# zhoupengwei/tloam

Hardware: AMD Instinct MI355X
Metric: gauss_newton_iters_per_sec (higher is better)
Workload: dtype f64

## Files before the change

tloam_amd/csrc/tl_gn.hip:

```cpp
#include <stdlib.h>
#include <string.h>

#include <hip/hip_ext.h>

#include "tl_common.hpp"
#include "tl_finish.hpp"

namespace tl {

struct Acc {
  double v[27];
  double pm;
  int pe;
};

__host__ __device__ constexpr int ut(int i, int j) { return i * 6 - (i * (i - 1)) / 2 + (j - i); }

__device__ __forceinline__ double fast_rcp(double x) {
  double r = __builtin_amdgcn_rcp(x);
  return __builtin_fma(r, __builtin_fma(-x, r, 1.0), r);
}
__device__ __forceinline__ double fast_rsqrt(double x) {
  double y = __builtin_amdgcn_rsq(x);
  const double h = 0.5 * x * y;
// ... 688 lines not shown
__device__ __forceinline__ void load_state_words(const GnState* st, GnState* sm) {
  constexpr int kWords = (int)(sizeof(GnState) / 8);
  static_assert(kWords <= 256, "one word per thread");
  if (threadIdx.x < kWords)
    reinterpret_cast<unsigned long long*>(sm)[threadIdx.x] = reinterpret_cast<const unsigned long long*>(st)[threadIdx.x];
}
__device__ __forceinline__ void stop_comm_error(GnState* st) {
  if (threadIdx.x == 0) { st->done = 1; st->comm_error = 1; }
}
__device__ __forceinline__ bool mbox_receive(const MboxView& mb, unsigned long long id, double* out , int count, int lane) {
  const bool ok = mbox_gather(mb, id, out, count, lane);
  if (lane == 0) {
    mb.ctr[0] = id;
    if (!ok) mb.ctr[1] = 1ull;
  }
  return ok;
}
__global__ __launch_bounds__(64) void k_gn_step(GnState* st, const double* __restrict__ in48, unsigned long long* iter_span) {
  __shared__ double tot[kReduceBuf];
  __shared__ double scr[32];
  __shared__ GnState s_in;
  if (threadIdx.x < kReduceBuf) tot[threadIdx.x] = in48[threadIdx.x];
  load_state_lds(st, &s_in, threadIdx.x);
  __syncthreads();
  if (s_in.done) return;
  const bool first = s_in.phase == PH_ITER0;
  gn_consume(st, tot, threadIdx.x, &s_in, scr);
  if (threadIdx.x == 0) iter_span_note(iter_span, first);
}
void launch_gn_step(GnState* st, const double* in48, hipStream_t s, unsigned long long* iter_span) {
  hipLaunchKernelGGL(k_gn_step, dim3(1), dim3(64), 0, s, st, in48, iter_span);
}
__global__ __launch_bounds__(64) void k_gn_step_mbox(GnState* st, MboxView mb, unsigned long long* iter_span) {
  __shared__ double tot[kMboxSlot];
  __shared__ double scr[32];
  __shared__ GnState s_in;
  load_state_lds(st, &s_in, threadIdx.x);
  __syncthreads();
  if (s_in.done) return;
  const bool ok = mbox_receive(mb, mbox_next_id(mb), tot, kReduceBuf, threadIdx.x);
  __syncthreads();
  if (!ok) {
    stop_comm_error(st);
    return;
  }
  const bool first = s_in.phase == PH_ITER0;
  gn_consume(st, tot, threadIdx.x, &s_in, scr);
  if (threadIdx.x == 0) iter_span_note(iter_span, first);
}
void launch_gn_step_mbox(GnState* st, const MboxView& mb, hipStream_t s, unsigned long long* iter_span) {
  hipLaunchKernelGGL(k_gn_step_mbox, dim3(1), dim3(64), 0, s, st, mb, iter_span);
}
__global__ __launch_bounds__(64) void k_mbox_gather_only(double* out48, MboxView mb) {
  __shared__ double tot[kMboxSlot];
  mbox_receive(mb, mbox_next_id(mb), tot, kReduceBuf, threadIdx.x);
  if (threadIdx.x < kReduceBuf) out48[threadIdx.x] = tot[threadIdx.x];
}
void launch_mbox_gather_only(double* out48, const MboxView& mb, hipStream_t s) {
  hipLaunchKernelGGL(k_mbox_gather_only, dim3(1), dim3(64), 0, s, out48, mb);
}
__global__ __launch_bounds__(64) void k_mbox_allreduce(double* buf, int count, MboxView mb) {
  __shared__ double vals[kMboxSlot];
  const int t = threadIdx.x;
  if (t < count) vals[t] = buf[t];
  __syncthreads();
  const unsigned long long id = mbox_next_id(mb);
  mbox_post(mb, id, vals, count, t);
  mbox_receive(mb, id, vals, count, t);
  __syncthreads();
  if (t < count) buf[t] = vals[t];
}
void launch_mbox_allreduce(double* buf, int count, const MboxView& mb, hipStream_t s) {
  hipLaunchKernelGGL(k_mbox_allreduce, dim3(1), dim3(64), 0, s, buf, count, mb);
}

__global__ __launch_bounds__(kRedThreads) void k_reduce_and_step(const double* __restrict__ partials, int rows,
                                                                 GnState* __restrict__ st, unsigned long long* iter_span) {
  __shared__ double lds[8 * 33];
  __shared__ double tot[kReduceBuf];
  __shared__ GnState s_in;
#ifdef TLOAM_STEP_PROFILE
  if (threadIdx.x == 0) st->dbg[0] = (double)__builtin_readcyclecounter();
#endif
  load_state_words(st, &s_in);
#ifdef TLOAM_STEP_PROFILE
  asm volatile("s_waitcnt vmcnt(0)" ::: "memory");
  if (threadIdx.x == 0) st->dbg[7] = (double)__builtin_readcyclecounter();
#endif
  fold_rows<false, 4>(partials, rows, lds, tot);
#ifdef TLOAM_STEP_PROFILE
  if (threadIdx.x == 0) st->dbg[8] = (double)__builtin_readcyclecounter();
#endif
  if (s_in.done) return;
  const bool first = s_in.phase == PH_ITER0;
  if (threadIdx.x < 64) gn_consume(st, tot, threadIdx.x, &s_in, lds );
  if (threadIdx.x == 0) iter_span_note(iter_span, first);
#ifdef TLOAM_STEP_PROFILE
  if (threadIdx.x == 0) st->dbg[6] = (double)__builtin_readcyclecounter();
#endif
}
struct K3Step {
  int* ticket;
  unsigned long long* span;
  unsigned long long* iter_span;
  MboxView mb;
};
template <bool SINGLE, int W = 4>
__global__ __launch_bounds__(64 * W, 2) void k3_sweep_step(const double* __restrict__ seg0, int stride0, int cap0, int unused,
                                                        GnState* __restrict__ st, const int* __restrict__ seg_n,
                                                        double* __restrict__ partials, CorrView cv, K3Step fs) {
  __shared__ double red[W][32];
  __shared__ double s_grp[8 * 33];
  __shared__ double tot[kMboxSlot];
  __shared__ GnState s_in;
  SweepStamps ts;
  sweep_body<SINGLE, W, false>(seg0, stride0, cap0, (unused & 2) != 0 , false, st, seg_n, cv, red,
                               ts, [&] {
    if (fs.span && blockIdx.x == 0 && threadIdx.x == 0)
      __hip_atomic_store(fs.span, (unsigned long long)wall_clock64(), __ATOMIC_RELAXED, __HIP_MEMORY_SCOPE_AGENT);
    load_state_words(st, &s_in);
  }, [&] {
    if (!k3_take_ticket<W>(partials, red, fs.ticket)) return;
    if (fs.span && threadIdx.x == 0) {
      const unsigned long long t1 = wall_clock64();
      const unsigned long long t0 = __hip_atomic_load(fs.span, __ATOMIC_RELAXED, __HIP_MEMORY_SCOPE_AGENT);
      fs.span[1] += t1 - t0;
      fs.span[2] += 1ull;
    }
    fold_rows<true>(partials, (int)gridDim.x, s_grp, tot);
    if (threadIdx.x == 0) __hip_atomic_store(fs.ticket, 0, __ATOMIC_RELAXED, __HIP_MEMORY_SCOPE_AGENT);
    if (threadIdx.x >= 64) return;
    if (fs.mb.nranks > 0) {
      const unsigned long long id = mbox_next_id(fs.mb);
      mbox_post(fs.mb, id, tot, kReduceBuf, (int)threadIdx.x);
      const bool ok = mbox_receive(fs.mb, id, tot, kReduceBuf, (int)threadIdx.x);
      asm volatile("s_waitcnt lgkmcnt(0)" ::: "memory");
      if (!ok) {
        stop_comm_error(st);
        return;
      }
    }
    const bool first = s_in.phase == PH_ITER0;
    gn_consume(st, tot, (int)threadIdx.x, &s_in, s_grp );
    if (threadIdx.x == 0) iter_span_note(fs.iter_span, first);
  });
}
void launch_k3_step(const CorrView& cv, GnState* st, double* partials, int grid, bool single, bool wide, int* ticket, unsigned long long* span,
                    const MboxView* mb_or_null, hipStream_t s, hipEvent_t ev_start, hipEvent_t ev_stop, unsigned long long* iter_span) {
  auto kern = single ? k3_sweep_step<true> : wide ? k3_sweep_step<false, 8> : k3_sweep_step<false>;
  K3Step fs;
  memset(&fs, 0, sizeof(fs));
  fs.ticket = ticket;
  fs.span = span;
  fs.iter_span = iter_span;
  if (mb_or_null) fs.mb = *mb_or_null;
  launch_sweep(kern, grid, wide ? 512 : 256, s, ev_start, ev_stop, cv, 0, st, partials, cv, fs);
}

__global__ __launch_bounds__(256, 1) void k_sweep_step_small(const double* __restrict__ seg0, int stride0, int cap0, int tagged,
                                                             GnState* __restrict__ st, const int* __restrict__ seg_n,
                                                             double* __restrict__ partials, int* __restrict__ ticket,
                                                             CorrView cv, unsigned long long* iter_span) {
  __shared__ double red[4][32];
  __shared__ double s_grp[8 * 33];
  __shared__ double s_rows[kTaggedRows * 28];
  __shared__ double tot[kReduceBuf];
  __shared__ GnState s_in;
  const int lane = threadIdx.x & 63, wave = __builtin_amdgcn_readfirstlane(threadIdx.x >> 6);
  const int gw = blockIdx.x * 4 + wave;
#ifdef TLOAM_STEP_PROFILE
  const unsigned long long c_entry = __builtin_readcyclecounter();
#endif
  ChunkData pre;
  const SingleWork wk = single_work_of(cv, cap0, gw, lane);
  const bool w2 = (tagged & 2) != 0;
  tagged &= 1;
  single_fetch(cv, seg0, stride0, wk, pre, w2);
  {
    constexpr int kWords = (int)(sizeof(GnState) / 8);
    static_assert(kWords <= 256, "one word per thread");
    if (threadIdx.x < kWords)
      reinterpret_cast<unsigned long long*>(&s_in)[threadIdx.x] = reinterpret_cast<const unsigned long long*>(st)[threadIdx.x];
  }
  unsigned long long* const epoch = reinterpret_cast<unsigned long long*>(ticket + 2);
  const unsigned long long epoch0 = *epoch;
  if (st->done) return;
  const Rt T = st->Rt_eval;
#ifdef TLOAM_STEP_PROFILE
  asm volatile("s_waitcnt lgkmcnt(0)" ::: "memory");
  const unsigned long long c_pose = __builtin_readcyclecounter();
#endif
  Acc a;
  sweep_single(cv, seg_n, T, wk, pre, a);
#ifdef TLOAM_STEP_PROFILE
  const unsigned long long c_eval = __builtin_readcyclecounter();
#endif
  const double wtot = wave_reduce_acc(a, lane);
  if ((lane & 1) == 0) red[wave][lane >> 1] = wtot;
  __syncthreads();
#ifdef TLOAM_STEP_PROFILE
  const unsigned long long c_sweep = __builtin_readcyclecounter();
#endif
  if (tagged) {
    k3_post_row_tagged(partials, red, epoch0 + 1ull);
    if (blockIdx.x != 0 || threadIdx.x >= 64) return;
#ifdef TLOAM_STEP_PROFILE
    if (threadIdx.x == 0) {
      st->dbg[7] = (double)c_sweep; st->dbg[0] = (double)__builtin_readcyclecounter();
      st->dbg[8] = (double)c_entry; st->dbg[9] = (double)c_pose; st->dbg[10] = (double)c_eval;
    }
#endif
    const bool ok = poll_fold_tagged(partials, (int)gridDim.x, epoch0 + 1ull, s_rows, tot, (int)threadIdx.x);
    if (threadIdx.x == 0) *epoch = epoch0 + 1ull;
    if (!ok) {
      if (threadIdx.x == 0) { st->done = 1; st->comm_error = 1; }
      return;
    }
  } else {
    if (!k3_take_ticket(partials, red, ticket)) return;
#ifdef TLOAM_STEP_PROFILE
    if (threadIdx.x == 0) { st->dbg[7] = (double)c_sweep; st->dbg[0] = (double)__builtin_readcyclecounter(); }
#endif
    fold_rows<true>(partials, (int)gridDim.x, s_grp, tot);
    if (threadIdx.x == 0) __hip_atomic_store(ticket, 0, __ATOMIC_RELAXED, __HIP_MEMORY_SCOPE_AGENT);
  }
  const bool first = s_in.phase == PH_ITER0;
  if (threadIdx.x < 64) gn_consume(st, tot, threadIdx.x, &s_in, s_grp );
  if (threadIdx.x == 0) iter_span_note(iter_span, first);
#ifdef TLOAM_STEP_PROFILE
  if (threadIdx.x == 0) st->dbg[6] = (double)__builtin_readcyclecounter();
#endif
}
void launch_sweep_step_small(const CorrView& cv, GnState* st, double* partials, int* ticket, int grid, hipStream_t s,
                             unsigned long long* iter_span) {
  launch_sweep(k_sweep_step_small, grid, 256, s, nullptr, nullptr, cv, grid <= kTaggedRows ? 1 : 0 , st, partials, ticket, cv,
               iter_span);
}
#include "tl_prep.hpp"

__device__ __forceinline__ bool weight_out_of_range(const WeightParams& wp, int kind, double c) {
  if (!wp.active[kind]) return false;
  if (c == 0) return false;
  if (c >= wp.th1 || c <= wp.th2) return false;
  if (c < wp.th1 * (1.0 - 1e-9) && c > wp.th2 * (1.0 + 1e-9)) return false;
  const double w = sqrt(wp.noise_bound_sq * wp.mu * (wp.mu + 1) / c) - wp.mu;
  return !(w >= 0.0 && w <= 1.0);
}
constexpr int kExtRowBase = 512;
__device__ __forceinline__ void post_ext_segment(double* __restrict__ partials, int gw, double cs, double bad, int kind, unsigned long long tag,
                                                 int lane, int base_word = kExtRowBase) {
  if (lane >= 8) return;
  unsigned long long wd = 0ull;
  const double cs0 = rdlane(cs, 0), bad0 = rdlane(bad, 0);
  if (lane == 0) wd = (unsigned long long)__double_as_longlong(cs0);
  else if (lane == 1) wd = (unsigned long long)__double_as_longlong(bad0);
  else if (lane == 2) wd = (unsigned long long)(long long)kind;
  const unsigned long long x = xor8(lane < 7 ? seg_word(wd, lane) : 0ull);
  if (lane == 7) wd = check_mix(tag) ^ x;
  __hip_atomic_store(reinterpret_cast<unsigned long long*>(partials) + base_word + (size_t)gw * 8 + lane, wd, __ATOMIC_RELAXED,
                     __HIP_MEMORY_SCOPE_AGENT);
}
__device__ __forceinline__ bool poll_fold_ext(const double* __restrict__ partials, int nwaves, unsigned long long tag, double* s_ext ,
                                              double* fin , int lane, int base_word = kExtRowBase) {
  const bool have = lane >= 1 && lane < nwaves;
  const unsigned long long mtag = check_mix(tag);
  const unsigned long long* p = reinterpret_cast<const unsigned long long*>(partials) + base_word + (size_t)(have ? lane : 1) * 8;
  unsigned long long w[8];
  const unsigned long long t0 = wall_clock64();
  bool ok_all;
  for (unsigned spins = 1;; ++spins) {
#pragma unroll
    for (int i = 0; i < 8; ++i) w[i] = __hip_atomic_load(p + i, __ATOMIC_RELAXED, __HIP_MEMORY_SCOPE_AGENT);
    unsigned long long x = w[7];
#pragma unroll
    for (int i = 0; i < 7; ++i) x ^= seg_word(w[i], i);
    ok_all = __all((!have || x == mtag) ? 1 : 0) != 0;
    if (ok_all) break;
    if ((spins & 63u) == 0 && wall_clock64() - t0 > 100000000ull) break;
    __builtin_amdgcn_s_sleep(1);
  }
  const double cs = have ? __longlong_as_double((long long)w[0]) : 0.0;
  const double bad = have ? __longlong_as_double((long long)w[1]) : 0.0;
  const int kind = have ? (int)(long long)w[2] : -1;
  double t[5];
#pragma unroll
  for (int k = 0; k < 4; ++k) t[k] = kind == k ? cs : 0.0;
  t[4] = bad;
#pragma unroll
  for (int off = 32; off > 0; off >>= 1)
#pragma unroll
    for (int k = 0; k < 5; ++k) t[k] += __shfl_down(t[k], off, 64);
  if (lane == 0) {
#pragma unroll
    for (int k = 0; k < 5; ++k) fin[k] = t[k];
  }
  asm volatile("s_waitcnt lgkmcnt(0)" ::: "memory");
  (void)s_ext;
  return ok_all;
}

__device__ __forceinline__ int finish_by_consumer(GnState* st, GnState* sm , const SolveFinish& F, int oi,
                                                  const double* fin, const int nseg[kKinds], double* sh , int lane,
                                                  bool lead = true) {
  constexpr int kWords = (int)(offsetof(GnState, dbg) / 8);
  const OuterCtl ctl{F.cost_threshold, 1, oi == F.n_iter - 1 ? 1 : 0};
  int next = 4;
  if (!sm->done) {
    if (lane == 0) {
      sm->incomplete = OS_INCOMPLETE;
      sm->stop = 2;
      sm->run_build = sm->run_refresh = 0;
    }
  } else {
    if (lane < 16) {
      double v = 0.0;
      if (lane < 4) v = fin[lane];
      else if (lane < 8) v = (double)(lane == 4 ? nseg[0] : (lane == 5 ? nseg[1] : (lane == 6 ? nseg[2] : nseg[3])));
      else if (lane == 8) v = fin[4];
      sh[lane] = v;
      if (lead) F.sums16[lane] = v;
    }
    asm volatile("s_waitcnt lgkmcnt(0)" ::: "memory");
    publish_and_rearm(sh, sm, lane, ctl);
    asm volatile("s_waitcnt lgkmcnt(0)" ::: "memory");
    next = (sm->stop == 0 && sm->run_build == 0 && sm->run_refresh != 0 && oi + 1 < F.n_iter) ? 3 : 4;
  }
  asm volatile("s_waitcnt lgkmcnt(0)" ::: "memory");
  if (!lead) return next;
  for (int w = lane; w < kWords; w += 64) reinterpret_cast<unsigned long long*>(st)[w] = reinterpret_cast<const unsigned long long*>(sm)[w];
  mirror_wave(sm, F.hm[oi], lane, (sm->stop == 0 && next == 4) ? (int)(sm->incomplete | OS_NEEDS_HOST) : -1);
  if (sm->stop != 0)
    for (int j = oi + 1; j < F.n_iter; ++j) mirror_wave(sm, F.hm[j], lane, (int)OS_SKIPPED);
  return next;
}

constexpr int kAllRowsParity = kTaggedRows * kAccStride;
constexpr int kAllExtBase = 2 * kAllRowsParity;
constexpr int kAllExtParity = 64 * 8;
__device__ __forceinline__ bool next_is_failure(const double* s_msg) {
  asm volatile("s_waitcnt lgkmcnt(0)" ::: "memory");
  return (int)s_msg[12] == 5;
}
__global__ __launch_bounds__(256, 1) void k_solve_all(const double* __restrict__ seg0, int stride0, int cap0, int max_sweeps,
                                                      GnState* __restrict__ st, const int* __restrict__ seg_n,
                                                      double* __restrict__ partials, int* __restrict__ ticket, CorrView cv, SolvePrep prep,
                                                      int* __restrict__ seg_n_out, SolveFinish F) {
  __shared__ double red[4][32];
  __shared__ double s_scr[32];
  __shared__ double s_rows[kTaggedRows * 28];
  __shared__ double s_ext[64 * 3];
  __shared__ double s_fin[8];
  __shared__ double s_sh[16];
  __shared__ double tot[kReduceBuf];
  __shared__ double s_msg[16];
  __shared__ GnState s_in;
  const int lane = threadIdx.x & 63, wave = __builtin_amdgcn_readfirstlane(threadIdx.x >> 6);
  const int gw = blockIdx.x * 4 + wave;
  const bool stepper = wave == 0;
  const bool lead = blockIdx.x == 0;
  const bool self_prep = prep.sv.flagb != nullptr;
  const unsigned long long sabotage = ((max_sweeps >> 16) & 1) ? (1ull << 40) : 0ull;
  max_sweeps &= 0xffff;
  unsigned long long* const epoch = reinterpret_cast<unsigned long long*>(ticket + 2);
#ifdef TLOAM_STEP_PROFILE
  unsigned long long* const prof = reinterpret_cast<unsigned long long*>(partials) + 2048;
  const bool prof_c = lead && stepper && lane == 0;
  const bool prof_p = (int)blockIdx.x == (int)gridDim.x / 2 && wave == 1 && lane == 0;
#define TL_PROF(cond, slot) if (cond) prof[(slot)] = wall_clock64();
#else
#define TL_PROF(cond, slot)
#endif
  ChunkData pre;
  const SingleWork wk = single_work_of(cv, cap0, gw, lane);
  single_fetch(cv, seg0, stride0, wk, pre);
  FlagBytes fbytes;
  if (self_prep && wk.kind >= 0) load_flag_bytes(prep.sv.flagb, wk.kind, lane, fbytes);
  if (stepper) {
    constexpr int kWords = (int)(sizeof(GnState) / 8);
    for (int w = lane; w < kWords; w += 64)
      reinterpret_cast<unsigned long long*>(&s_in)[w] = reinterpret_cast<const unsigned long long*>(st)[w];
  }
  const unsigned long long tag0 = (*epoch + 1ull) << 8;
  int oi = F.first_iter;
  if (F.enabled && (st->stop != 0 || st->next_outer != oi)) return;
  const bool build = self_prep && (!prep.run_build || *prep.run_build != 0);
  const bool refresh = self_prep && !build && prep.run_refresh && *prep.run_refresh != 0;
  const bool done_at_entry = st->done != 0;
  Rt T = st->Rt_eval;
  int n_mine = 0;
  int slot[2] = {0, 0};
  int nseg[kKinds] = {0, 0, 0, 0};
  if (lead && stepper) {
    if (build) {
      FlagBytes fb[kKinds];
#pragma unroll
      for (int k = 0; k < kKinds; ++k) load_flag_bytes(prep.sv.flagb, k, lane, fb[k]);
#pragma unroll
      for (int k = 0; k < kKinds; ++k) nseg[k] = kind_set_of(prep, cv, k, lane, fb[k]).total;
      if (lane < kKinds) seg_n_out[lane] = lane == 0 ? nseg[0] : (lane == 1 ? nseg[1] : (lane == 2 ? nseg[2] : nseg[3]));
    } else {
#pragma unroll
      for (int k = 0; k < kKinds; ++k) nseg[k] = seg_n[k];
    }
  }
  if (wk.kind >= 0) {
    if (build) {
      n_mine = self_compact(prep, cv, wk, lane, fbytes, pre, slot);
    } else {
      n_mine = seg_n[wk.kind];
      if (self_prep) {
        slots_of_chunk(prep, cv, wk, n_mine, slot);
        if (refresh) self_refresh(prep, cv, wk, n_mine, slot, pre);
      }
    }
  }
  if (stepper) {
    asm volatile("s_waitcnt vmcnt(0) lgkmcnt(0)" ::: "memory");
    if (build && lane < 6) {
      s_in.x_build[lane] = s_in.x[lane];
      if (lead) st->x_build[lane] = s_in.x[lane];
    }
  }
  if (done_at_entry) return;
  TL_PROF(prof_c, 0)
  unsigned long long h = 0;
  for (;;) {
    int verdict = 2;
    double2 last_cost = double2{0.0, 0.0};
    for (int it = 0;; ++it) {
      Acc a;
      last_cost = double2{0.0, 0.0};
      sweep_single_n(cv, n_mine, T, wk, pre, a, &last_cost);
      TL_PROF(prof_p, 64 + it * 8 + 1)
      const double wtot = wave_reduce_acc(a, lane);
      if ((lane & 1) == 0) red[wave][lane >> 1] = wtot;
      __syncthreads();
      double* const rows = partials + (size_t)(h & 1ull) * kAllRowsParity;
      const int ext_base = kAllExtBase + (int)(h & 1ull) * kAllExtParity;
      k3_post_row_tagged(rows, red, tag0 | h);
      TL_PROF(prof_c, 8 + it * 8 + 0)
      if (F.have_wp) {
        double cs = last_cost.x + last_cost.y;
        double bad = 0.0;
        if (wk.kind >= 0) {
          const bool two = single_chunk_of(wk.kind) == kChunk;
          if (wk.j < n_mine && weight_out_of_range(F.wp[oi], wk.kind, last_cost.x)) bad += 1.0;
          if (two && wk.j + 1 < n_mine && weight_out_of_range(F.wp[oi], wk.kind, last_cost.y)) bad += 1.0;
        }
#pragma unroll
        for (int off = 32; off > 0; off >>= 1) {
          cs += __shfl_down(cs, off, 64);
          bad += __shfl_down(bad, off, 64);
        }
        post_ext_segment(partials, gw, cs, bad, wk.kind, tag0 | h, lane, ext_base);
      }
      TL_PROF(prof_p, 64 + it * 8 + 2)
      if (stepper) {
        const bool ok = poll_fold_tagged(rows, (int)gridDim.x, (tag0 | h) ^ sabotage, s_rows, tot, lane);
        TL_PROF(prof_c, 8 + it * 8 + 1)
        int vd = 5;
        if (ok) {
          gn_consume(st, tot, lane, &s_in, s_scr, false);
          vd = (s_in.done == 0 && it + 1 < max_sweeps) ? 1 : 2;
          if (lead && lane == 0) iter_span_note(F.iter_span, it == 0);
        }
        TL_PROF(prof_c, 8 + it * 8 + 2)
        if (lane < 9) s_msg[lane] = s_in.Rt_eval.r[lane];
        else if (lane < 12) s_msg[lane] = s_in.Rt_eval.t[lane - 9];
        else if (lane == 12) s_msg[12] = (double)vd;
      }
      __syncthreads();
      verdict = (int)s_msg[12];
      if (lead && stepper && verdict != 5) gn_write_back(st, &s_in, lane);
#pragma unroll
      for (int v = 0; v < 9; ++v) T.r[v] = s_msg[v];
#pragma unroll
      for (int v = 0; v < 3; ++v) T.t[v] = s_msg[9 + v];
      TL_PROF(prof_c, 8 + it * 8 + 3)
      TL_PROF(prof_p, 64 + (it + 1) * 8 + 0)
      h += 1ull;
      if (verdict != 1) break;
    }
    if (verdict == 5) {
      if (lead && stepper) {
        if (lane == 0) {
          st->done = 1; st->comm_error = 1;
          s_in.done = 1; s_in.comm_error = 1;
          if (F.enabled) {
            s_in.incomplete = OS_COMM_ERROR;
            st->incomplete = OS_COMM_ERROR;
            st->stop = 1; st->run_build = 0; st->run_refresh = 0;
          }
          *epoch = tag0 >> 8;
        }
        asm volatile("s_waitcnt lgkmcnt(0)" ::: "memory");
        if (F.enabled) {
          mirror_wave(&s_in, F.hm[oi], lane, (int)OS_COMM_ERROR);
          for (int j = oi + 1; j < F.n_iter; ++j) mirror_wave(&s_in, F.hm[j], lane, (int)OS_SKIPPED);
        }
      }
      return;
    }
    double2 w_new = pre.w;
    if (F.enabled && wk.kind >= 0) {
      const bool two = single_chunk_of(wk.kind) == kChunk;
      if (wk.j < n_mine) w_new.x = refreshed_weight(F.wp[oi], wk.kind, last_cost.x, pre.w.x, prep.sv.w_src, slot[0]);
      if (two && wk.j + 1 < n_mine) w_new.y = refreshed_weight(F.wp[oi], wk.kind, last_cost.y, pre.w.y, prep.sv.w_src, slot[1]);
    }
    if (stepper) {
      int next = 4;
      bool ok = true;
      if (F.have_wp)
        ok = poll_fold_ext(partials, (int)gridDim.x * 4, tag0 | (h - 1ull), s_ext, s_fin, lane, kAllExtBase + (int)((h - 1ull) & 1ull) * kAllExtParity);
      if (!ok) {
        next = 5;
      } else if (!F.enabled) {
        if (lead) {
          if (F.have_wp && lane < 5) {
            const double v = s_fin[lane];
            if (lane < 4) st->fin_sum[lane] = v; else st->fin_bad = v;
          }
          if (lane == 0) { st->fin_valid = F.have_wp ? 1 : 0; *epoch = tag0 >> 8; }
        }
      } else {
        next = finish_by_consumer(st, &s_in, F, oi, s_fin, nseg, s_sh, lane, lead);
      }
      if (lane < 9) s_msg[lane] = s_in.Rt_eval.r[lane];
      else if (lane < 12) s_msg[lane] = s_in.Rt_eval.t[lane - 9];
      else if (lane == 12) s_msg[12] = (double)next;
    }
    if (!F.enabled) {
      if (lead && stepper && next_is_failure(s_msg) && lane == 0) {
        st->done = 1; st->comm_error = 1; s_in.done = 1; s_in.comm_error = 1;
        st->fin_valid = 0;
        *epoch = tag0 >> 8;
      }
      return;
    }
    __syncthreads();
    const int next = (int)s_msg[12];
#pragma unroll
    for (int v = 0; v < 9; ++v) T.r[v] = s_msg[v];
#pragma unroll
    for (int v = 0; v < 3; ++v) T.t[v] = s_msg[9 + v];
    if (next == 5) {
      if (lead && stepper) {
        if (lane == 0) {
          st->done = 1; st->comm_error = 1; s_in.done = 1; s_in.comm_error = 1;
          s_in.incomplete = OS_COMM_ERROR; st->incomplete = OS_COMM_ERROR;
          st->stop = 1; st->run_build = 0; st->run_refresh = 0;
          *epoch = tag0 >> 8;
        }
        asm volatile("s_waitcnt lgkmcnt(0)" ::: "memory");
        mirror_wave(&s_in, F.hm[oi], lane, (int)OS_COMM_ERROR);
        for (int j = oi + 1; j < F.n_iter; ++j) mirror_wave(&s_in, F.hm[j], lane, (int)OS_SKIPPED);
      }
      return;
    }
    if (next != 3) {
      if (lead && stepper && lane == 0) *epoch = tag0 >> 8;
      return;
    }
    if (wk.kind >= 0) {
      const CorrSeg& seg = cv.k[wk.kind];
      const bool two = single_chunk_of(wk.kind) == kChunk;
      pre.w = w_new;
      if (wk.j < n_mine) { seg.w[wk.j] = w_new.x; seg.cost[wk.j] = 0.0; }
      if (two && wk.j + 1 < n_mine) { seg.w[wk.j + 1] = w_new.y; seg.cost[wk.j + 1] = 0.0; }
    }
    oi += 1;
  }
}
void launch_solve_small(const CorrView& cv, GnState* st, double* partials, int* ticket, int grid, int max_sweeps,
                        const SolvePrep* prep_or_null, int* seg_n, const SolveFinish* finish_or_null, hipStream_t s) {
  SolvePrep P;
  if (prep_or_null) P = *prep_or_null;
  else memset(&P, 0, sizeof(P));
  SolveFinish F;
  if (finish_or_null) F = *finish_or_null;
  else memset(&F, 0, sizeof(F));
  hipLaunchKernelGGL(k_solve_all, dim3(grid), dim3(256), 0, s, (const double*)cv.k[0].px, cv.k[0].stride, cv.k[0].cap, max_sweeps, st,
                     cv.seg_n, partials, ticket, cv, P, seg_n, F);
}
void launch_reduce_and_step(const double* partials, int grid, GnState* st, hipStream_t s, unsigned long long* iter_span) {
  hipLaunchKernelGGL(k_reduce_and_step, dim3(1), dim3(kRedThreads), 0, s, partials, grid, st, iter_span);
}

__global__ void k_debug_se3(const double* __restrict__ x, const double* __restrict__ delta, int n, double* __restrict__ out) {
  const int i = blockIdx.x * blockDim.x + threadIdx.x;
  if (i >= n) return;
  double xv[6], dv[6];
#pragma unroll
  for (int k = 0; k < 6; ++k) { xv[k] = x[6 * i + k]; dv[k] = delta[6 * i + k]; }
  const Pose E = exp_fast2(dv);
  const Pose X = exp_fast2(xv);
  double lx[6], pl[6];
  log_fast2(X, lx);
  log_fast2(compose_fast2(E, X), pl);
  const Pose X2 = se3_exp(xv);
  double* o = out + 26 * (size_t)i;
  o[0] = E.qw; o[1] = E.qx; o[2] = E.qy; o[3] = E.qz; o[4] = E.tx; o[5] = E.ty; o[6] = E.tz;
#pragma unroll
  for (int k = 0; k < 6; ++k) { o[7 + k] = lx[k]; o[13 + k] = pl[k]; }
  o[19] = X2.qw; o[20] = X2.qx; o[21] = X2.qy; o[22] = X2.qz; o[23] = X2.tx; o[24] = X2.ty; o[25] = X2.tz;
}
void launch_debug_se3(const double* x, const double* delta, int n, double* out, hipStream_t s) {
  hipLaunchKernelGGL(k_debug_se3, dim3((n + 63) / 64), dim3(64), 0, s, x, delta, n, out);
}

__global__ __launch_bounds__(256) void k_weights(WeightArgs A, double* __restrict__ partial, const GnState* __restrict__ st) {
  __shared__ double red[4][8];
  if (!st->done || st->stop) return;
  double sum[kKinds] = {0, 0, 0, 0};
  double bad = 0.0;
  const int tid = blockIdx.x * 256 + threadIdx.x, stride = gridDim.x * 256;
#pragma unroll
  for (int k = 0; k < kKinds; ++k) {
    const int n = A.cv.seg_n[k];
    const CorrSeg& seg = A.cv.k[k];
    constexpr int kU = 4;
    for (int i0 = tid; i0 < n; i0 += kU * stride) {
      double cu[kU];
      int iu[kU];
#pragma unroll
      for (int u = 0; u < kU; ++u) {
        const int i = i0 + u * stride;
        cu[u] = (i < n) ? seg.cost[i] : 0.0;
        iu[u] = (i < n) ? seg.idx[i] : 0;
      }
#pragma unroll
      for (int u = 0; u < kU; ++u) {
        if (i0 + u * stride >= n) break;
        const double c = cu[u];
        sum[k] += c;
        if (!A.wp.active[k]) continue;
        if (c == 0) continue;
        double w;
        if (c >= A.wp.th1) w = 0.0;
        else if (c <= A.wp.th2) w = 1.0;
        else {
          w = sqrt(A.wp.noise_bound_sq * A.wp.mu * (A.wp.mu + 1) / c) - A.wp.mu;
          if (!(w >= 0.0 && w <= 1.0)) bad += 1.0;
        }
        const int slot = A.sv.slot_off[k] + (iu[u] - A.sv.src_lo[k]);
        A.sv.w_src[slot] = w;
      }
    }
  }
  double v[5] = {sum[0], sum[1], sum[2], sum[3], bad};
  const int lane = threadIdx.x & 63, wave = threadIdx.x >> 6;
#pragma unroll
  for (int i = 0; i < 5; ++i) {
#pragma unroll
    for (int off = 32; off > 0; off >>= 1) v[i] += __shfl_down(v[i], off, 64);
    if (lane == 0) red[wave][i] = v[i];
  }
  __syncthreads();
  if (threadIdx.x < 8) {
    double t = 0.0;
    if (threadIdx.x < 5) t = ((red[0][threadIdx.x] + red[1][threadIdx.x]) + red[2][threadIdx.x]) + red[3][threadIdx.x];
    partial[blockIdx.x * 8 + threadIdx.x] = t;
  }
}
void launch_weights(const CorrView& cv, const SlotView& sv, const WeightParams& wp, double* partial, int blocks,
                    const GnState* st, hipStream_t s) {
  WeightArgs A;
  A.cv = cv;
  A.sv = sv;
  A.wp = wp;
  hipLaunchKernelGGL(k_weights, dim3(blocks), dim3(256), 0, s, A, partial, st);
}

__global__ __launch_bounds__(64) void k_outer_finish(const double* __restrict__ partial, int blocks,
                                                     const int* __restrict__ seg_n, double* __restrict__ sums16,
                                                     GnState* st_or_null, GnState* gate, HostMirror hm, OuterCtl ctl) {
  __shared__ double sh[16];
  const int t = threadIdx.x;
  {
    const int g = finish_gate(gate, ctl, t);
    if (g != 0) {
      if (st_or_null) mirror_to_host(gate, hm, t, 64, g == 1 ? (int)OS_SKIPPED : -1);
      return;
    }
  }
  double v[5] = {0, 0, 0, 0, 0};
  for (int b = t; b < blocks; b += 64) {
#pragma unroll
    for (int c = 0; c < 5; ++c) v[c] += partial[b * 8 + c];
  }
#pragma unroll
  for (int c = 0; c < 5; ++c)
#pragma unroll
    for (int off = 32; off > 0; off >>= 1) v[c] += __shfl_down(v[c], off, 64);
  if (t < 16) sh[t] = 0.0;
  __syncthreads();
  if (t == 0) {
#pragma unroll
    for (int c = 0; c < 4; ++c) sh[c] = v[c];
    sh[8] = v[4];
  }
  if (t >= 4 && t < 8) sh[t] = (double)seg_n[t - 4];
  __syncthreads();
  if (t < 16) sums16[t] = sh[t];
  if (st_or_null) {
    publish_and_rearm(sh, st_or_null, t, ctl);
    mirror_to_host(st_or_null, hm, t, 64);
  }
}
void launch_outer_finish(const double* partial, int blocks, const int* seg_n, GnState* st_or_null, GnState* gate,
                         double* sums16, HostMirror hm, OuterCtl ctl, hipStream_t s) {
  hipLaunchKernelGGL(k_outer_finish, dim3(1), dim3(64), 0, s, partial, blocks, seg_n, sums16, st_or_null, gate, hm, ctl);
}
__global__ void k_outer_publish(const double* __restrict__ sums16, GnState* st, HostMirror hm,
                                const unsigned long long* __restrict__ comm_err) {
  if (st->done) publish_and_rearm(sums16, st, threadIdx.x, OuterCtl{0.0, 0, 0});
  if (threadIdx.x == 0 && (st->comm_error || (comm_err && *comm_err))) st->incomplete = 3;
  mirror_to_host(st, hm, threadIdx.x, 64);
}
void launch_outer_publish(const double* sums16, GnState* st, HostMirror hm, const unsigned long long* comm_err,
                          hipStream_t s) {
  hipLaunchKernelGGL(k_outer_publish, dim3(1), dim3(64), 0, s, sums16, st, hm, comm_err);
}

struct Mat16 { double m[16]; };
__global__ void k_transform(double* aos, size_t n, Mat16 M) {
  size_t i = (size_t)blockIdx.x * blockDim.x + threadIdx.x;
  const size_t stride = (size_t)gridDim.x * blockDim.x;
  for (; i < n; i += stride) {
    const double x = aos[3 * i], y = aos[3 * i + 1], z = aos[3 * i + 2];
    double o[4];
#pragma unroll
    for (int r = 0; r < 4; ++r) o[r] = M.m[r] * x + M.m[4 + r] * y + M.m[8 + r] * z + M.m[12 + r];
    aos[3 * i] = o[0] / o[3];
    aos[3 * i + 1] = o[1] / o[3];
    aos[3 * i + 2] = o[2] / o[3];
  }
}
void launch_transform_cloud(double* aos, size_t n, const double M[16], hipStream_t s) {
  if (n == 0) return;
  Mat16 m;
  for (int i = 0; i < 16; ++i) m.m[i] = M[i];
  int blocks = (int)((n + 255) / 256);
  if (blocks > 4096) blocks = 4096;
  hipLaunchKernelGGL(k_transform, dim3(blocks), dim3(256), 0, s, aos, n, m);
}

}
```

Before: 63850.

## Fold weight-check partials early on a helper wave and defer state write-out

Wave 1 now waits on a workgroup flag until the stepper has folded the row partials, then folds the ext-segment cost/bad partials into a separate shared buffer while the stepper runs its inner solve. The stepper uses these early results in the outer finish instead of polling the ext segments again. The GnState copy and mirror write-out is split out of finish_by_consumer and, when the outer loop continues, runs after the barrier that releases the other waves rather than before it. This adds spin-waiting on a helper wave and extra profiling hooks, and it risks ordering problems around the early-fold flag.

```diff
diff --git a/tloam_amd/csrc/tl_gn.hip b/tloam_amd/csrc/tl_gn.hip
--- a/tloam_amd/csrc/tl_gn.hip
+++ b/tloam_amd/csrc/tl_gn.hip
@@ -1014,7 +1014,6 @@
 __device__ __forceinline__ int finish_by_consumer(GnState* st, GnState* sm , const SolveFinish& F, int oi,
                                                   const double* fin, const int nseg[kKinds], double* sh , int lane,
                                                   bool lead = true) {
-  constexpr int kWords = (int)(offsetof(GnState, dbg) / 8);
   const OuterCtl ctl{F.cost_threshold, 1, oi == F.n_iter - 1 ? 1 : 0};
   int next = 4;
   if (!sm->done) {
@@ -1038,12 +1037,15 @@
     next = (sm->stop == 0 && sm->run_build == 0 && sm->run_refresh != 0 && oi + 1 < F.n_iter) ? 3 : 4;
   }
   asm volatile("s_waitcnt lgkmcnt(0)" ::: "memory");
-  if (!lead) return next;
+  return next;
+}
+__device__ __forceinline__ void finish_write_out(GnState* st, const GnState* sm , const SolveFinish& F, int oi,
+                                                 int next, int lane) {
+  constexpr int kWords = (int)(offsetof(GnState, dbg) / 8);
   for (int w = lane; w < kWords; w += 64) reinterpret_cast<unsigned long long*>(st)[w] = reinterpret_cast<const unsigned long long*>(sm)[w];
   mirror_wave(sm, F.hm[oi], lane, (sm->stop == 0 && next == 4) ? (int)(sm->incomplete | OS_NEEDS_HOST) : -1);
   if (sm->stop != 0)
     for (int j = oi + 1; j < F.n_iter; ++j) mirror_wave(sm, F.hm[j], lane, (int)OS_SKIPPED);
-  return next;
 }
 
 constexpr int kAllRowsParity = kTaggedRows * kAccStride;
@@ -1062,6 +1064,9 @@
   __shared__ double s_rows[kTaggedRows * 28];
   __shared__ double s_ext[64 * 3];
   __shared__ double s_fin[8];
+  __shared__ double s_fin_early[8];
+  __shared__ unsigned long long s_early_h;
+  __shared__ unsigned long long s_rows_h;
   __shared__ double s_sh[16];
   __shared__ double tot[kReduceBuf];
   __shared__ double s_msg[16];
@@ -1078,9 +1083,12 @@
   unsigned long long* const prof = reinterpret_cast<unsigned long long*>(partials) + 2048;
   const bool prof_c = lead && stepper && lane == 0;
   const bool prof_p = (int)blockIdx.x == (int)gridDim.x / 2 && wave == 1 && lane == 0;
+  constexpr int kProfEnd = 256;
 #define TL_PROF(cond, slot) if (cond) prof[(slot)] = wall_clock64();
+#define TL_PROF_VAL(cond, slot, val) if (cond) prof[(slot)] = (unsigned long long)(val);
 #else
 #define TL_PROF(cond, slot)
+#define TL_PROF_VAL(cond, slot, val)
 #endif
   ChunkData pre;
   const SingleWork wk = single_work_of(cv, cap0, gw, lane);
@@ -1134,6 +1142,8 @@
     }
   }
   if (done_at_entry) return;
+  if (wave == 1 && lane == 0) s_early_h = 0ull;
+  if (stepper && lane == 0) s_rows_h = 0ull;
   TL_PROF(prof_c, 0)
   unsigned long long h = 0;
   for (;;) {
@@ -1151,6 +1161,7 @@
       const int ext_base = kAllExtBase + (int)(h & 1ull) * kAllExtParity;
       k3_post_row_tagged(rows, red, tag0 | h);
       TL_PROF(prof_c, 8 + it * 8 + 0)
+      TL_PROF(prof_c && it == 0 && oi > F.first_iter, kProfEnd + 16 * (oi - 1) + 5)
       if (F.have_wp) {
         double cs = last_cost.x + last_cost.y;
         double bad = 0.0;
@@ -1165,10 +1176,22 @@
           bad += __shfl_down(bad, off, 64);
         }
         post_ext_segment(partials, gw, cs, bad, wk.kind, tag0 | h, lane, ext_base);
+        if (wave == 1) {
+          const unsigned long long t0 = wall_clock64();
+          __builtin_amdgcn_s_sleep(40);
+          for (unsigned spins = 1; __hip_atomic_load(&s_rows_h, __ATOMIC_RELAXED, __HIP_MEMORY_SCOPE_WORKGROUP) != h + 1ull; ++spins) {
+            if ((spins & 63u) == 0 && wall_clock64() - t0 > 200000000ull) break;
+            __builtin_amdgcn_s_sleep(4);
+          }
+          const bool got = poll_fold_ext(partials, (int)gridDim.x * 4, tag0 | h, s_ext, s_fin_early, lane, ext_base);
+          if (lane == 0) s_early_h = got ? h + 1ull : 0ull;
+          TL_PROF((lead && lane == 0), kProfEnd + 16 * oi + 10)
+        }
       }
       TL_PROF(prof_p, 64 + it * 8 + 2)
       if (stepper) {
         const bool ok = poll_fold_tagged(rows, (int)gridDim.x, (tag0 | h) ^ sabotage, s_rows, tot, lane);
+        if (lane == 0) __hip_atomic_store(&s_rows_h, h + 1ull, __ATOMIC_RELAXED, __HIP_MEMORY_SCOPE_WORKGROUP);
         TL_PROF(prof_c, 8 + it * 8 + 1)
         int vd = 5;
         if (ok) {
@@ -1222,20 +1245,31 @@
     if (stepper) {
       int next = 4;
       bool ok = true;
-      if (F.have_wp)
+      TL_PROF(prof_c, kProfEnd + 16 * oi + 0)
+      TL_PROF_VAL(prof_c, kProfEnd + 16 * oi + 8, s_in.spec_build)
+      TL_PROF_VAL(prof_c, kProfEnd + 16 * oi + 9, tag0)
+      const bool early = F.have_wp && s_early_h == h;
+      const double* const fin = early ? s_fin_early : s_fin;
+      if (F.have_wp && !early)
         ok = poll_fold_ext(partials, (int)gridDim.x * 4, tag0 | (h - 1ull), s_ext, s_fin, lane, kAllExtBase + (int)((h - 1ull) & 1ull) * kAllExtParity);
+      TL_PROF_VAL(prof_c, kProfEnd + 16 * oi + 11, early ? 1 : 0)
+      TL_PROF(prof_c, kProfEnd + 16 * oi + 1)
       if (!ok) {
         next = 5;
       } else if (!F.enabled) {
         if (lead) {
           if (F.have_wp && lane < 5) {
-            const double v = s_fin[lane];
+            const double v = fin[lane];
             if (lane < 4) st->fin_sum[lane] = v; else st->fin_bad = v;
           }
           if (lane == 0) { st->fin_valid = F.have_wp ? 1 : 0; *epoch = tag0 >> 8; }
         }
       } else {
-        next = finish_by_consumer(st, &s_in, F, oi, s_fin, nseg, s_sh, lane, lead);
+        next = finish_by_consumer(st, &s_in, F, oi, fin, nseg, s_sh, lane, lead);
+        TL_PROF(prof_c, kProfEnd + 16 * oi + 2)
+        if (lead && next != 3) finish_write_out(st, &s_in, F, oi, next, lane);
+        TL_PROF(prof_c && next != 3, kProfEnd + 16 * oi + 3)
+        TL_PROF_VAL(prof_c, kProfEnd + 16 * oi + 6, next)
       }
       if (lane < 9) s_msg[lane] = s_in.Rt_eval.r[lane];
       else if (lane < 12) s_msg[lane] = s_in.Rt_eval.t[lane - 9];
@@ -1250,6 +1284,7 @@
       return;
     }
     __syncthreads();
+    TL_PROF(prof_c, kProfEnd + 16 * oi + 4)
     const int next = (int)s_msg[12];
 #pragma unroll
     for (int v = 0; v < 9; ++v) T.r[v] = s_msg[v];
@@ -1271,7 +1306,12 @@
     }
     if (next != 3) {
       if (lead && stepper && lane == 0) *epoch = tag0 >> 8;
+      TL_PROF(prof_c, kProfEnd + 16 * oi + 7)
       return;
+    }
+    if (lead && stepper) {
+      finish_write_out(st, &s_in, F, oi, 3, lane);
+      TL_PROF(prof_c, kProfEnd + 16 * oi + 3)
     }
     if (wk.kind >= 0) {
       const CorrSeg& seg = cv.k[wk.kind];
```

Result: slower. 63150 (-1.1%).
